# phonism/genrec

Measured on NVIDIA H100. Metric: hstu_train_sequences_per_sec, higher is better.
Workload: dtype bf16

## Files before the change

genrec_b200/csrc/tc_ce.cuh:

```cuda
#pragma once
#include "tc_gemm.cuh"

namespace grb {

template <int TB>
GRB_DEVINL void wgmma_m64n64k16_ss(float (&d)[32], uint64_t adesc, uint64_t bdesc, uint32_t accumulate) {
    asm volatile(
        "{\n"
        ".reg .pred p;\n"
        "setp.ne.b32 p, %34, 0;\n"
        "wgmma.mma_async.sync.aligned.m64n64k16.f32.bf16.bf16 {%0,%1,%2,%3,%4,%5,%6,%7,%8,%9,%10,%11,%12,%13,%14,%15,%16,%17,%18,%19,%20,%21,%22,%23,%24,%25,%26,%27,%28,%29,%30,%31}, %32, %33, p, 1, 1, 0, %35;\n"
        "}\n"
        : "+f"(d[0]), "+f"(d[1]), "+f"(d[2]), "+f"(d[3]), "+f"(d[4]), "+f"(d[5]), "+f"(d[6]), "+f"(d[7]), "+f"(d[8]), "+f"(d[9]), "+f"(d[10]), "+f"(d[11]), "+f"(d[12]), "+f"(d[13]), "+f"(d[14]), "+f"(d[15]), "+f"(d[16]), "+f"(d[17]), "+f"(d[18]), "+f"(d[19]), "+f"(d[20]), "+f"(d[21]), "+f"(d[22]), "+f"(d[23]), "+f"(d[24]), "+f"(d[25]), "+f"(d[26]), "+f"(d[27]), "+f"(d[28]), "+f"(d[29]), "+f"(d[30]), "+f"(d[31])
        : "l"(adesc), "l"(bdesc), "r"(accumulate), "n"(TB));
}
template <int TB>
GRB_DEVINL void wgmma_m64n64k16_rs(float (&d)[32], const uint32_t (&a)[4], uint64_t bdesc, uint32_t accumulate) {
    asm volatile(
        "{\n"
        ".reg .pred p;\n"
        "setp.ne.b32 p, %37, 0;\n"
        "wgmma.mma_async.sync.aligned.m64n64k16.f32.bf16.bf16 {%0,%1,%2,%3,%4,%5,%6,%7,%8,%9,%10,%11,%12,%13,%14,%15,%16,%17,%18,%19,%20,%21,%22,%23,%24,%25,%26,%27,%28,%29,%30,%31}, {%32,%33,%34,%35}, %36, p, 1, 1, %38;\n"
        "}\n"
        : "+f"(d[0]), "+f"(d[1]), "+f"(d[2]), "+f"(d[3]), "+f"(d[4]), "+f"(d[5]), "+f"(d[6]), "+f"(d[7]), "+f"(d[8]), "+f"(d[9]), "+f"(d[10]), "+f"(d[11]), "+f"(d[12]), "+f"(d[13]), "+f"(d[14]), "+f"(d[15]), "+f"(d[16]), "+f"(d[17]), "+f"(d[18]), "+f"(d[19]), "+f"(d[20]), "+f"(d[21]), "+f"(d[22]), "+f"(d[23]), "+f"(d[24]), "+f"(d[25]), "+f"(d[26]), "+f"(d[27]), "+f"(d[28]), "+f"(d[29]), "+f"(d[30]), "+f"(d[31])
        : "r"(a[0]), "r"(a[1]), "r"(a[2]), "r"(a[3]), "l"(bdesc), "r"(accumulate), "n"(TB));
}
template <int TB>
GRB_DEVINL void wgmma_m64n128k16_rs(float (&d)[64], const uint32_t (&a)[4], uint64_t bdesc, uint32_t accumulate) {
    asm volatile(
        "{\n"
        ".reg .pred p;\n"
        "setp.ne.b32 p, %69, 0;\n"
        "wgmma.mma_async.sync.aligned.m64n128k16.f32.bf16.bf16 {%0,%1,%2,%3,%4,%5,%6,%7,%8,%9,%10,%11,%12,%13,%14,%15,%16,%17,%18,%19,%20,%21,%22,%23,%24,%25,%26,%27,%28,%29,%30,%31,%32,%33,%34,%35,%36,%37,%38,%39,%40,%41,%42,%43,%44,%45,%46,%47,%48,%49,%50,%51,%52,%53,%54,%55,%56,%57,%58,%59,%60,%61,%62,%63}, {%64,%65,%66,%67}, %68, p, 1, 1, %70;\n"
        "}\n"
        : "+f"(d[0]), "+f"(d[1]), "+f"(d[2]), "+f"(d[3]), "+f"(d[4]), "+f"(d[5]), "+f"(d[6]), "+f"(d[7]), "+f"(d[8]), "+f"(d[9]), "+f"(d[10]), "+f"(d[11]), "+f"(d[12]), "+f"(d[13]), "+f"(d[14]), "+f"(d[15]), "+f"(d[16]), "+f"(d[17]), "+f"(d[18]), "+f"(d[19]), "+f"(d[20]), "+f"(d[21]), "+f"(d[22]), "+f"(d[23]), "+f"(d[24]), "+f"(d[25]), "+f"(d[26]), "+f"(d[27]), "+f"(d[28]), "+f"(d[29]), "+f"(d[30]), "+f"(d[31]), "+f"(d[32]), "+f"(d[33]), "+f"(d[34]), "+f"(d[35]), "+f"(d[36]), "+f"(d[37]), "+f"(d[38]), "+f"(d[39]), "+f"(d[40]), "+f"(d[41]), "+f"(d[42]), "+f"(d[43]), "+f"(d[44]), "+f"(d[45]), "+f"(d[46]), "+f"(d[47]), "+f"(d[48]), "+f"(d[49]), "+f"(d[50]), "+f"(d[51]), "+f"(d[52]), "+f"(d[53]), "+f"(d[54]), "+f"(d[55]), "+f"(d[56]), "+f"(d[57]), "+f"(d[58]), "+f"(d[59]), "+f"(d[60]), "+f"(d[61]), "+f"(d[62]), "+f"(d[63])
        : "r"(a[0]), "r"(a[1]), "r"(a[2]), "r"(a[3]), "l"(bdesc), "r"(accumulate), "n"(TB));
}

template <int D>
GRB_DEVINL void wgmma_rs_d(float (&d)[D / 2], const uint32_t (&a)[4], uint64_t bdesc) {
    if constexpr (D == 64) wgmma_m64n64k16_rs<1>(d, a, bdesc, 1u);
    else wgmma_m64n128k16_rs<1>(d, a, bdesc, 1u);
}

constexpr int CE_THREADS = 384;
constexpr int CE_STAGES = 4;
constexpr float CE_L2E = 1.4426950408889634f;
constexpr int CE_MAX_SEGMENTS = 8;

struct CeArgs {
    const long long* tg;
    const float* inv_count;
    int T, C;
    float* dx;
    float* shift;
    float* row_loss;
    float* dtable;
    int rseg, tseg;
    int* rsched;
    int* tsched;
    float* rcarry;
    float* tcarry;
};

inline int ce_segments(int items, int span, int sms) {
    const int cap = span < CE_MAX_SEGMENTS ? span : CE_MAX_SEGMENTS;
    int best = 1;
    long long best_n = 0, best_slots = 1;
    for (int s = 1; s <= cap; ++s) {
        const long long n = (long long)items * s, slots = (n + sms - 1) / sms * sms;
        if (16 * n >= 15 * slots) return s;
        if (n * best_slots > best_n * slots) { best = s; best_n = n; best_slots = slots; }
    }
    return best;
}
inline int ce_row_segments(int T, int C, int sms) { return ce_segments(2 * ((T + 127) / 128), (C + 63) / 64, sms); }
inline int ce_table_segments(int T, int C, int sms) { return ce_segments((C + 63) / 64, (T + 63) / 64, sms); }

template <int D>
struct CeSmem {
    static constexpr int XB = D / 64;
    static constexpr int ROW_TILE = XB * 128 * 128;
    static constexpr int CLS_TILE = XB * 64 * 128;
    static constexpr int ROWS_BYTES = ROW_TILE + CE_STAGES * CLS_TILE + 1024 + 256;
    static constexpr int TABLE_BYTES = CLS_TILE + CE_STAGES * CLS_TILE + 1024 + 256;
};

GRB_DEVINL void ce_bar(int id, int n) { asm volatile("bar.sync %0, %1;" ::"r"(id), "r"(n) : "memory"); }
GRB_DEVINL void ce_wait_chain(const int* flag, int need) {
    if (threadIdx.x == 128) {
        int v;
        do asm volatile("ld.acquire.gpu.global.s32 %0, [%1];" : "=r"(v) : "l"(flag) : "memory");
        while (v < need);
    }
    ce_bar(2, 256);
}
GRB_DEVINL void ce_finish_segment(int* flag) {
    __threadfence();
    ce_bar(2, 256);
    if (threadIdx.x == 128) atomicAdd(flag, 1);
}

template <int D>
GRB_DEVINL void ce_scores(float (&S)[32], uint32_t a_addr, int a_box, uint32_t b_addr) {
    wgmma_fence();
#pragma unroll
    for (int kk = 0; kk < D / 16; ++kk)
        wgmma_m64n64k16_ss<0>(S, wgmma_desc(a_addr + (kk >> 2) * a_box + (kk & 3) * 32, 16, 1024),
                              wgmma_desc(b_addr + (kk >> 2) * 8192 + (kk & 3) * 32, 16, 1024), kk > 0 ? 1u : 0u);
    wgmma_commit();
    wgmma_wait<0>();
}
template <int D>
GRB_DEVINL void ce_accumulate(float (&acc)[D / 2], const float (&G)[32], uint32_t b_addr) {
    uint32_t a[4][4];
#pragma unroll
    for (int kk = 0; kk < 4; ++kk) {
        a[kk][0] = pack_bf16(G[8 * kk], G[8 * kk + 1]);
        a[kk][1] = pack_bf16(G[8 * kk + 2], G[8 * kk + 3]);
        a[kk][2] = pack_bf16(G[8 * kk + 4], G[8 * kk + 5]);
        a[kk][3] = pack_bf16(G[8 * kk + 6], G[8 * kk + 7]);
    }
    wgmma_fence();
#pragma unroll
    for (int kk = 0; kk < 4; ++kk) wgmma_rs_d<D>(acc, a[kk], wgmma_desc(b_addr + kk * 2048, 8192, 1024));
    wgmma_commit();
    wgmma_wait<0>();
}

struct CeCta {
    unsigned char* stat;
    unsigned char* ring;
    uint64_t *full, *empty;
    uint64_t* sfull;
    unsigned char* tail;
};
template <int D>
GRB_DEVINL CeCta ce_cta_init(unsigned char* raw, int stat_bytes, int empty_arrivals, const CUtensorMap* tmX, const CUtensorMap* tmE) {
    CeCta cta;
    cta.stat = raw + ((1024u - (smem_u32(raw) & 1023u)) & 1023u);
    cta.ring = cta.stat + stat_bytes;
    cta.full = reinterpret_cast<uint64_t*>(cta.ring + CE_STAGES * CeSmem<D>::CLS_TILE);
    cta.empty = cta.full + CE_STAGES;
    cta.sfull = cta.full + 2 * CE_STAGES;
    cta.tail = cta.ring + CE_STAGES * CeSmem<D>::CLS_TILE + 256;
    if (threadIdx.x == 0) {
        tma_prefetch_desc(tmX);
        tma_prefetch_desc(tmE);
        for (int s = 0; s < CE_STAGES; ++s) { mbar_init(&cta.full[s], 1); mbar_init(&cta.empty[s], empty_arrivals); }
        mbar_init(cta.sfull, 1);
        fence_barrier_init();
    }
    __syncthreads();
    pdl_wait();
    return cta;
}
template <int D, int ROWS>
GRB_DEVINL void ce_tile_load(const CeCta& cta, const CUtensorMap* tm, int row0) {
    mbar_expect_tx(cta.sfull, D / 64 * ROWS * 128);
    for (int b = 0; b < D / 64; ++b) tma_load_2d(cta.stat + b * ROWS * 128, tm, b * 64, row0, cta.sfull);
}
template <int D>
GRB_DEVINL void ce_ring_load(const CeCta& cta, const CUtensorMap* tm, int row0, int stage, uint32_t empty_parity) {
    mbar_wait(&cta.empty[stage], empty_parity);
    mbar_expect_tx(&cta.full[stage], CeSmem<D>::CLS_TILE);
    for (int b = 0; b < D / 64; ++b) tma_load_2d(cta.ring + stage * CeSmem<D>::CLS_TILE + b * 8192, tm, b * 64, row0, &cta.full[stage]);
}

struct CeLane {
    int g, w, q, lane;
    bool leader;
    GRB_DEVINL int row(int base, int i) const { return base + 16 * w + (lane >> 2) + 8 * i; }
};
GRB_DEVINL CeLane ce_lane() {
    const int warp = threadIdx.x >> 5, lane = threadIdx.x & 31;
    return CeLane{(warp >> 2) - 1, warp & 3, lane & 3, lane, (threadIdx.x & 127) == 0};
}

GRB_DEVINL void ce_softmax_step(const float (&S)[32], int i, float& m, float& s) {
    float mx = -INFINITY;
#pragma unroll
    for (int jj = 0; jj < 8; ++jj)
#pragma unroll
        for (int c = 0; c < 2; ++c) mx = fmaxf(mx, S[jj * 4 + i * 2 + c]);
    mx = fmaxf(mx, __shfl_xor_sync(0xffffffffu, mx, 1));
    mx = fmaxf(mx, __shfl_xor_sync(0xffffffffu, mx, 2));
    const float mn = fmaxf(m, mx);
    float acc = s * ex2_fast((m - mn) * CE_L2E);
#pragma unroll
    for (int jj = 0; jj < 8; ++jj)
#pragma unroll
        for (int c = 0; c < 2; ++c) acc += ex2_fast((S[jj * 4 + i * 2 + c] - mn) * CE_L2E);
    s = acc;
    m = mn;
}
GRB_DEVINL float ce_row_finish(float m, float s, float& lse) {
    s += __shfl_xor_sync(0xffffffffu, s, 1);
    s += __shfl_xor_sync(0xffffffffu, s, 2);
    lse = m + __logf(s);
    return m * CE_L2E + __log2f(s);
}

struct CeCols {
    int tg[16];
    float sh[16], icc[16];
};
template <class Target>
GRB_DEVINL void ce_table_cols(CeCols& k, const CeLane& l, int tt, int T, const float* shift, float inv, Target target) {
#pragma unroll
    for (int jj = 0; jj < 8; ++jj)
#pragma unroll
        for (int c = 0; c < 2; ++c) {
            const int t = tt * 64 + 8 * jj + 2 * l.q + c;
            const bool ok = t < T;
            k.tg[jj * 2 + c] = ok ? target(t) : 0;
            k.sh[jj * 2 + c] = ok ? shift[t] : 0.f;
            k.icc[jj * 2 + c] = k.tg[jj * 2 + c] != 0 ? inv : 0.f;
        }
}
template <int D>
GRB_DEVINL void ce_wg_handover(const CeCta& cta, const CeLane& l, const float (&acc)[D / 2]) {
    float* red = reinterpret_cast<float*>(cta.ring);
    ce_bar(2, 256);
    if (l.g == 1) {
#pragma unroll
        for (int kk = 0; kk < D / 2; ++kk) red[(size_t)kk * 128 + (threadIdx.x & 127)] = acc[kk];
    }
    ce_bar(2, 256);
}
GRB_DEVINL float ce_wg_peer(const CeCta& cta, int kk) { return reinterpret_cast<const float*>(cta.ring)[(size_t)kk * 128 + (threadIdx.x & 127)]; }

template <int D>
__global__ void __launch_bounds__(CE_THREADS, 1)
    ce_rows_kernel(const __grid_constant__ CUtensorMap tmX, const __grid_constant__ CUtensorMap tmE, CeArgs a) {
    using SM = CeSmem<D>;
    extern __shared__ unsigned char ce_smem_raw[];
    __shared__ int unit_slot[2];
    const CeCta cta = ce_cta_init<D>(ce_smem_raw, SM::ROW_TILE, 2, &tmX, &tmE);
    const int warp = threadIdx.x >> 5, lane = threadIdx.x & 31;
    if (warp >= 1 && warp < 4) return;
    const int ntile = (a.C + 63) / 64, R = (a.T + 127) / 128, K = a.rseg;
    const int units = (a.dx ? 2 : 1) * K * R;
    const CeLane l = ce_lane();
    const int q = l.q;
    int stage = 0;
    uint32_t phase = 0;
    for (int n = 0;; ++n) {
        if (threadIdx.x == 0) unit_slot[n & 1] = atomicAdd(a.rsched, 1);
        ce_bar(1, 288);
        const int u = unit_slot[n & 1];
        if (u >= units) break;
        const bool dxp = u >= K * R;
        const int k = u / R % K, rt = u % R, row0 = rt * 128;
        const int j0 = k * ntile / K, j1 = (k + 1) * ntile / K;
        int* sdone = a.rsched + 1 + rt;
        int* xdone = a.rsched + 1 + R + rt;
        if (warp == 0) {
            if (lane == 0) {
                ce_tile_load<D, 128>(cta, &tmX, row0);
                for (int j = j0; j < j1; ++j) {
                    ce_ring_load<D>(cta, &tmE, j * 64, stage, phase ^ 1);
                    if (++stage == CE_STAGES) { stage = 0; phase ^= 1; }
                }
            }
            __syncwarp();
            continue;
        }
        int row[2], tgt[2];
        float ic[2];
        const float inv = *a.inv_count;
#pragma unroll
        for (int i = 0; i < 2; ++i) {
            row[i] = l.row(row0 + 64 * l.g, i);
            tgt[i] = row[i] < a.T ? (int)a.tg[row[i]] : 0;
            ic[i] = tgt[i] != 0 ? inv : 0.f;
        }
        mbar_wait(cta.sfull, n & 1);
        const uint32_t xa = smem_u32(cta.stat) + l.g * 8192;
        if (!dxp) {
            if (k > 0) ce_wait_chain(sdone, k);
            float m[2] = {-INFINITY, -INFINITY}, s[2] = {0.f, 0.f}, tl[2] = {0.f, 0.f};
            const size_t plane = (size_t)a.T * 4;
#pragma unroll
            for (int i = 0; i < 2; ++i)
                if (k > 0 && row[i] < a.T) {
                    const size_t at = (size_t)row[i] * 4 + q;
                    m[i] = __ldcg(a.rcarry + at);
                    s[i] = __ldcg(a.rcarry + plane + at);
                    tl[i] = __ldcg(a.rcarry + 2 * plane + at);
                }
            for (int j = j0; j < j1; ++j) {
                mbar_wait(&cta.full[stage], phase);
                float S[32];
                ce_scores<D>(S, xa, 16384, smem_u32(cta.ring + stage * SM::CLS_TILE));
                if (l.leader) mbar_arrive(&cta.empty[stage]);
                if (++stage == CE_STAGES) { stage = 0; phase ^= 1; }
#pragma unroll
                for (int i = 0; i < 2; ++i) {
#pragma unroll
                    for (int jj = 0; jj < 8; ++jj)
#pragma unroll
                        for (int c = 0; c < 2; ++c) {
                            const int col = j * 64 + 8 * jj + 2 * q + c;
                            float& v = S[jj * 4 + i * 2 + c];
                            if (col >= a.C) v = -INFINITY;
                            if (col == tgt[i]) tl[i] = v;
                        }
                    ce_softmax_step(S, i, m[i], s[i]);
                }
            }
            if (k + 1 < K) {
#pragma unroll
                for (int i = 0; i < 2; ++i)
                    if (row[i] < a.T) {
                        const size_t at = (size_t)row[i] * 4 + q;
                        a.rcarry[at] = m[i];
                        a.rcarry[plane + at] = s[i];
                        a.rcarry[2 * plane + at] = tl[i];
                    }
            } else {
#pragma unroll
                for (int i = 0; i < 2; ++i) {
                    float lse;
                    const float shift = ce_row_finish(m[i], s[i], lse);
                    tl[i] += __shfl_xor_sync(0xffffffffu, tl[i], 1);
                    tl[i] += __shfl_xor_sync(0xffffffffu, tl[i], 2);
                    if (q == 0 && row[i] < a.T) {
                        a.row_loss[row[i]] = tgt[i] != 0 ? (lse - tl[i]) * ic[i] : 0.f;
                        a.shift[row[i]] = shift;
                    }
                }
            }
            ce_finish_segment(sdone);
        } else {
            if (k > 0) ce_wait_chain(xdone, k);
            else ce_wait_chain(sdone, K);
            float shift[2];
#pragma unroll
            for (int i = 0; i < 2; ++i) shift[i] = row[i] < a.T ? __ldcg(a.shift + row[i]) : 0.f;
            float dx[D / 2];
#pragma unroll
            for (int jj = 0; jj < D / 8; ++jj)
#pragma unroll
                for (int i = 0; i < 2; ++i) {
                    float2 v = make_float2(0.f, 0.f);
                    if (k > 0 && row[i] < a.T) v = __ldcg(reinterpret_cast<const float2*>(a.dx + (size_t)row[i] * D + 8 * jj + 2 * q));
                    dx[jj * 4 + i * 2] = v.x;
                    dx[jj * 4 + i * 2 + 1] = v.y;
                }
            for (int j = j0; j < j1; ++j) {
                mbar_wait(&cta.full[stage], phase);
                float S[32];
                const uint32_t e_addr = smem_u32(cta.ring + stage * SM::CLS_TILE);
                ce_scores<D>(S, xa, 16384, e_addr);
#pragma unroll
                for (int jj = 0; jj < 8; ++jj)
#pragma unroll
                    for (int i = 0; i < 2; ++i)
#pragma unroll
                        for (int c = 0; c < 2; ++c) {
                            const int col = j * 64 + 8 * jj + 2 * q + c;
                            float& v = S[jj * 4 + i * 2 + c];
                            float gv = col < a.C ? ex2_fast(v * CE_L2E - shift[i]) * ic[i] : 0.f;
                            if (col == tgt[i]) gv -= ic[i];
                            v = gv;
                        }
                ce_accumulate<D>(dx, S, e_addr);
                if (l.leader) mbar_arrive(&cta.empty[stage]);
                if (++stage == CE_STAGES) { stage = 0; phase ^= 1; }
            }
#pragma unroll
            for (int jj = 0; jj < D / 8; ++jj)
#pragma unroll
                for (int i = 0; i < 2; ++i)
                    if (row[i] < a.T)
                        *reinterpret_cast<float2*>(a.dx + (size_t)row[i] * D + 8 * jj + 2 * q) = make_float2(dx[jj * 4 + i * 2], dx[jj * 4 + i * 2 + 1]);
            ce_finish_segment(xdone);
        }
    }
}

template <int D>
__global__ void __launch_bounds__(CE_THREADS, 1)
    ce_table_kernel(const __grid_constant__ CUtensorMap tmX, const __grid_constant__ CUtensorMap tmE, CeArgs a) {
    using SM = CeSmem<D>;
    extern __shared__ unsigned char ce_smem_raw[];
    __shared__ int unit_slot[2];
    const CeCta cta = ce_cta_init<D>(ce_smem_raw, SM::CLS_TILE, 1, &tmX, &tmE);
    const int warp = threadIdx.x >> 5, lane = threadIdx.x & 31;
    if (warp >= 1 && warp < 4) return;
    const int ntt = (a.T + 63) / 64, NC = (a.C + 63) / 64, K = a.tseg;
    const CeLane l = ce_lane();
    const int g = l.g, q = l.q;
    uint32_t pos = 0;
    for (int n = 0;; ++n) {
        if (threadIdx.x == 0) unit_slot[n & 1] = atomicAdd(a.tsched, 1);
        ce_bar(1, 288);
        const int u = unit_slot[n & 1];
        if (u >= K * NC) break;
        const int k = u / NC, ct = u % NC, cls0 = ct * 64;
        const int t0 = k * ntt / K, t1 = (k + 1) * ntt / K;
        int* done = a.tsched + 1 + ct;
        if (warp == 0) {
            if (lane == 0) {
                ce_tile_load<D, 64>(cta, &tmE, cls0);
                for (int tt = t0; tt < t1; ++tt) {
                    const uint32_t p = pos + (tt - t0);
                    ce_ring_load<D>(cta, &tmX, tt * 64, p % CE_STAGES, ((p / CE_STAGES) & 1) ^ 1);
                }
            }
            __syncwarp();
            pos += t1 - t0;
            continue;
        }
        const int cls[2] = {l.row(cls0, 0), l.row(cls0, 1)};
        const float inv = *a.inv_count;
        float acc[D / 2];
        float* carry = a.tcarry + ((size_t)ct * 2 + g) * (D / 2) * 128 + (threadIdx.x & 127);
        if (k > 0) ce_wait_chain(done, k);
#pragma unroll
        for (int kk = 0; kk < D / 2; ++kk) acc[kk] = k > 0 ? __ldcg(carry + (size_t)kk * 128) : 0.f;
        mbar_wait(cta.sfull, n & 1);
        const uint32_t ea = smem_u32(cta.stat);
        for (int tt = t0 + ((t0 ^ g) & 1); tt < t1; tt += 2) {
            const uint32_t p = pos + (tt - t0);
            const int stage = p % CE_STAGES;
            CeCols col;
            ce_table_cols(col, l, tt, a.T, a.shift, inv, [&](int t) { return (int)a.tg[t]; });
            mbar_wait(&cta.full[stage], (p / CE_STAGES) & 1);
            const uint32_t x_addr = smem_u32(cta.ring + stage * SM::CLS_TILE);
            float S[32];
            ce_scores<D>(S, ea, 8192, x_addr);
#pragma unroll
            for (int jj = 0; jj < 8; ++jj)
#pragma unroll
                for (int i = 0; i < 2; ++i)
#pragma unroll
                    for (int c = 0; c < 2; ++c) {
                        float& v = S[jj * 4 + i * 2 + c];
                        const int kq = jj * 2 + c;
                        float gv = ex2_fast(v * CE_L2E - col.sh[kq]) * col.icc[kq];
                        if (cls[i] == col.tg[kq]) gv -= col.icc[kq];
                        v = gv;
                    }
            ce_accumulate<D>(acc, S, x_addr);
            if (l.leader) mbar_arrive(&cta.empty[stage]);
        }
        pos += t1 - t0;
        if (k + 1 < K) {
#pragma unroll
            for (int kk = 0; kk < D / 2; ++kk) carry[(size_t)kk * 128] = acc[kk];
            ce_finish_segment(done);
            continue;
        }
        ce_wg_handover<D>(cta, l, acc);
        if (g == 0) {
#pragma unroll
            for (int jj = 0; jj < D / 8; ++jj)
#pragma unroll
                for (int i = 0; i < 2; ++i) {
                    const int c = l.row(cls0, i);
                    const int kk = jj * 4 + i * 2;
                    const float v0 = acc[kk] + ce_wg_peer(cta, kk), v1 = acc[kk + 1] + ce_wg_peer(cta, kk + 1);
                    if (c < a.C) {
                        float* dst = a.dtable + (size_t)c * D + 8 * jj + 2 * q;
                        atomicAdd(dst, v0);
                        atomicAdd(dst + 1, v1);
                    }
                }
        }
    }
}

template <int D>
inline cudaError_t launch_tc_ce(const bf16* xf, const bf16* table, const CeArgs& a, int ctas, cudaStream_t st) {
    CUtensorMap tmX, tmE;
    if (!make_tmap_bf16(&tmX, xf, a.T, D, D, 64, 128) || !make_tmap_bf16(&tmE, table, a.C, D, D, 64, 64)) return cudaErrorInvalidValue;
    cudaError_t e = set_max_smem(ce_rows_kernel<D>, CeSmem<D>::ROWS_BYTES);
    if (e != cudaSuccess) return e;
    const int R = (a.T + 127) / 128, units = (a.dx ? 2 : 1) * a.rseg * R;
    e = cudaMemsetAsync(a.rsched, 0, (size_t)(1 + 2 * R) * sizeof(int), st);
    if (e != cudaSuccess) return e;
    launch_k(ce_rows_kernel<D>, units < ctas ? units : ctas, CE_THREADS, CeSmem<D>::ROWS_BYTES, st, tmX, tmE, a);
    return cudaGetLastError();
}
template <int D>
inline cudaError_t launch_ce_table(const bf16* xf, const bf16* table, const CeArgs& a, int ctas, cudaStream_t st) {
    CUtensorMap tmX, tmE;
    if (!make_tmap_bf16(&tmX, xf, a.T, D, D, 64, 64) || !make_tmap_bf16(&tmE, table, a.C, D, D, 64, 64)) return cudaErrorInvalidValue;
    cudaError_t e = set_max_smem(ce_table_kernel<D>, CeSmem<D>::TABLE_BYTES);
    if (e != cudaSuccess) return e;
    const int NC = (a.C + 63) / 64, units = a.tseg * NC;
    e = cudaMemsetAsync(a.tsched, 0, (size_t)(1 + NC) * sizeof(int), st);
    if (e != cudaSuccess) return e;
    launch_k(ce_table_kernel<D>, units < ctas ? units : ctas, CE_THREADS, CeSmem<D>::TABLE_BYTES, st, tmX, tmE, a);
    return cudaGetLastError();
}

}
```

Measured before the change: 40610.

## Double-buffer CE score WGMMAs and split producer warp with register reallocation

Restructures the CE rows kernel so that the next tile's score WGMMA is issued before the current tile's softmax or gradient body runs, using two score register buffers and wait<1>. The producer warpgroup now shrinks its registers with setmaxnreg and loops independently, while the consumer warpgroups grow theirs. The aim is to hide tensor-core latency behind the exp and accumulation math. In exchange it raises register pressure and makes stage and phase tracking more complex through a shared position counter.

```diff
diff --git a/genrec_b200/csrc/tc_ce.cuh b/genrec_b200/csrc/tc_ce.cuh
--- a/genrec_b200/csrc/tc_ce.cuh
+++ b/genrec_b200/csrc/tc_ce.cuh
@@ -1,4 +1,5 @@
 #pragma once
+#include <type_traits>
 #include "tc_gemm.cuh"
 
 namespace grb {
@@ -44,6 +45,8 @@
 }
 
 constexpr int CE_THREADS = 384;
+constexpr int CE_PRODUCER_REGS = 40;
+constexpr int CE_CONSUMER_REGS = 232;
 constexpr int CE_STAGES = 4;
 constexpr float CE_L2E = 1.4426950408889634f;
 constexpr int CE_MAX_SEGMENTS = 8;
@@ -102,13 +105,17 @@
 }
 
 template <int D>
-GRB_DEVINL void ce_scores(float (&S)[32], uint32_t a_addr, int a_box, uint32_t b_addr) {
+GRB_DEVINL void ce_scores_issue(float (&S)[32], uint32_t a_addr, int a_box, uint32_t b_addr) {
     wgmma_fence();
 #pragma unroll
     for (int kk = 0; kk < D / 16; ++kk)
         wgmma_m64n64k16_ss<0>(S, wgmma_desc(a_addr + (kk >> 2) * a_box + (kk & 3) * 32, 16, 1024),
                               wgmma_desc(b_addr + (kk >> 2) * 8192 + (kk & 3) * 32, 16, 1024), kk > 0 ? 1u : 0u);
     wgmma_commit();
+}
+template <int D>
+GRB_DEVINL void ce_scores(float (&S)[32], uint32_t a_addr, int a_box, uint32_t b_addr) {
+    ce_scores_issue<D>(S, a_addr, a_box, b_addr);
     wgmma_wait<0>();
 }
 template <int D>
@@ -126,6 +133,34 @@
     for (int kk = 0; kk < 4; ++kk) wgmma_rs_d<D>(acc, a[kk], wgmma_desc(b_addr + kk * 2048, 8192, 1024));
     wgmma_commit();
     wgmma_wait<0>();
+}
+template <int N>
+GRB_DEVINL void setmaxnreg_dec() { asm volatile("setmaxnreg.dec.sync.aligned.u32 %0;" ::"n"(N)); }
+template <int N>
+GRB_DEVINL void setmaxnreg_inc() { asm volatile("setmaxnreg.inc.sync.aligned.u32 %0;" ::"n"(N)); }
+template <class Issue, class Body>
+GRB_DEVINL void ce_pipeline(int j0, int j1, int d, Issue&& issue, Body&& body) {
+    float Sa[32], Sb[32];
+    issue(Sa, j0);
+    for (int j = j0;; j += 2 * d) {
+        if (j + d >= j1) { body(Sa, j, std::true_type{}); return; }
+        issue(Sb, j + d);
+        body(Sa, j, std::false_type{});
+        if (j + 2 * d >= j1) { body(Sb, j + d, std::true_type{}); return; }
+        issue(Sa, j + 2 * d);
+        body(Sb, j + d, std::false_type{});
+    }
+}
+template <bool LAST>
+GRB_DEVINL void ce_wait_scores(std::integral_constant<bool, LAST>) { wgmma_wait<LAST ? 0 : 1>(); }
+GRB_DEVINL void ce_arrive_if(uint64_t* bar, bool pred) {
+    asm volatile(
+        "{\n"
+        ".reg .pred p;\n"
+        "setp.ne.b32 p, %1, 0;\n"
+        "@p mbarrier.arrive.shared::cta.b64 _, [%0];\n"
+        "}\n" ::"r"(smem_u32(bar)), "r"((int)pred)
+        : "memory");
 }
 
 struct CeCta {
@@ -237,16 +272,34 @@
     extern __shared__ unsigned char ce_smem_raw[];
     __shared__ int unit_slot[2];
     const CeCta cta = ce_cta_init<D>(ce_smem_raw, SM::ROW_TILE, 2, &tmX, &tmE);
-    const int warp = threadIdx.x >> 5, lane = threadIdx.x & 31;
-    if (warp >= 1 && warp < 4) return;
     const int ntile = (a.C + 63) / 64, R = (a.T + 127) / 128, K = a.rseg;
     const int units = (a.dx ? 2 : 1) * K * R;
+    if (threadIdx.x < 128) {
+        setmaxnreg_dec<CE_PRODUCER_REGS>();
+        if (threadIdx.x >= 32) return;
+        int stage = 0;
+        uint32_t phase = 0;
+        for (int n = 0;; ++n) {
+            if (threadIdx.x == 0) unit_slot[n & 1] = atomicAdd(a.rsched, 1);
+            ce_bar(1, 288);
+            const int u = unit_slot[n & 1];
+            if (u >= units) return;
+            const int k = u / R % K;
+            if (threadIdx.x == 0) {
+                ce_tile_load<D, 128>(cta, &tmX, u % R * 128);
+                for (int j = k * ntile / K; j < (k + 1) * ntile / K; ++j) {
+                    ce_ring_load<D>(cta, &tmE, j * 64, stage, phase ^ 1);
+                    if (++stage == CE_STAGES) { stage = 0; phase ^= 1; }
+                }
+            }
+            __syncwarp();
+        }
+    }
+    setmaxnreg_inc<CE_CONSUMER_REGS>();
     const CeLane l = ce_lane();
     const int q = l.q;
-    int stage = 0;
-    uint32_t phase = 0;
+    uint32_t pos = 0;
     for (int n = 0;; ++n) {
-        if (threadIdx.x == 0) unit_slot[n & 1] = atomicAdd(a.rsched, 1);
         ce_bar(1, 288);
         const int u = unit_slot[n & 1];
         if (u >= units) break;
@@ -255,17 +308,6 @@
         const int j0 = k * ntile / K, j1 = (k + 1) * ntile / K;
         int* sdone = a.rsched + 1 + rt;
         int* xdone = a.rsched + 1 + R + rt;
-        if (warp == 0) {
-            if (lane == 0) {
-                ce_tile_load<D, 128>(cta, &tmX, row0);
-                for (int j = j0; j < j1; ++j) {
-                    ce_ring_load<D>(cta, &tmE, j * 64, stage, phase ^ 1);
-                    if (++stage == CE_STAGES) { stage = 0; phase ^= 1; }
-                }
-            }
-            __syncwarp();
-            continue;
-        }
         int row[2], tgt[2];
         float ic[2];
         const float inv = *a.inv_count;
@@ -277,6 +319,13 @@
         }
         mbar_wait(cta.sfull, n & 1);
         const uint32_t xa = smem_u32(cta.stat) + l.g * 8192;
+        auto tile = [&](int j) { return smem_u32(cta.ring + (pos + (j - j0)) % CE_STAGES * SM::CLS_TILE); };
+        auto issue = [&](float (&S)[32], int j) {
+            const uint32_t p = pos + (j - j0);
+            mbar_wait(&cta.full[p % CE_STAGES], (p / CE_STAGES) & 1);
+            ce_scores_issue<D>(S, xa, 16384, tile(j));
+        };
+        auto release = [&](int j) { ce_arrive_if(&cta.empty[(pos + (j - j0)) % CE_STAGES], l.leader); };
         if (!dxp) {
             if (k > 0) ce_wait_chain(sdone, k);
             float m[2] = {-INFINITY, -INFINITY}, s[2] = {0.f, 0.f}, tl[2] = {0.f, 0.f};
@@ -289,12 +338,9 @@
                     s[i] = __ldcg(a.rcarry + plane + at);
                     tl[i] = __ldcg(a.rcarry + 2 * plane + at);
                 }
-            for (int j = j0; j < j1; ++j) {
-                mbar_wait(&cta.full[stage], phase);
-                float S[32];
-                ce_scores<D>(S, xa, 16384, smem_u32(cta.ring + stage * SM::CLS_TILE));
-                if (l.leader) mbar_arrive(&cta.empty[stage]);
-                if (++stage == CE_STAGES) { stage = 0; phase ^= 1; }
+            ce_pipeline(j0, j1, 1, issue, [&](float (&S)[32], int j, auto last) {
+                ce_wait_scores(last);
+                release(j);
 #pragma unroll
                 for (int i = 0; i < 2; ++i) {
 #pragma unroll
@@ -308,7 +354,8 @@
                         }
                     ce_softmax_step(S, i, m[i], s[i]);
                 }
-            }
+            });
+            pos += j1 - j0;
             if (k + 1 < K) {
 #pragma unroll
                 for (int i = 0; i < 2; ++i)
@@ -348,11 +395,8 @@
                     dx[jj * 4 + i * 2] = v.x;
                     dx[jj * 4 + i * 2 + 1] = v.y;
                 }
-            for (int j = j0; j < j1; ++j) {
-                mbar_wait(&cta.full[stage], phase);
-                float S[32];
-                const uint32_t e_addr = smem_u32(cta.ring + stage * SM::CLS_TILE);
-                ce_scores<D>(S, xa, 16384, e_addr);
+            ce_pipeline(j0, j1, 1, issue, [&](float (&S)[32], int j, auto last) {
+                ce_wait_scores(last);
 #pragma unroll
                 for (int jj = 0; jj < 8; ++jj)
 #pragma unroll
@@ -361,14 +405,15 @@
                         for (int c = 0; c < 2; ++c) {
                             const int col = j * 64 + 8 * jj + 2 * q + c;
                             float& v = S[jj * 4 + i * 2 + c];
-                            float gv = col < a.C ? ex2_fast(v * CE_L2E - shift[i]) * ic[i] : 0.f;
+                            float gv = ex2_fast(v * CE_L2E - shift[i]) * ic[i];
+                            if (col >= a.C) gv = 0.f;
                             if (col == tgt[i]) gv -= ic[i];
                             v = gv;
                         }
-                ce_accumulate<D>(dx, S, e_addr);
-                if (l.leader) mbar_arrive(&cta.empty[stage]);
-                if (++stage == CE_STAGES) { stage = 0; phase ^= 1; }
-            }
+                ce_accumulate<D>(dx, S, tile(j));
+                release(j);
+            });
+            pos += j1 - j0;
 #pragma unroll
             for (int jj = 0; jj < D / 8; ++jj)
 #pragma unroll
```

Result: faster. 41570 (median of 6 runs) (+2.4%).
